# nanoporetech/bonito

Measured on AMD Instinct MI355X. Metric: signal samples/sec/GPU (chunk=10000, batch=512) + read accuracy vs ref, higher is better.
Workload: dtype f16

## Files before the change

### bonito_amd/csrc/conv.hip

```cpp
#include "common.h"
#include "kernels.h"
#include "options.h"
#include <cstring>

namespace bh {

struct ConvFirstArgs {
    const half_t* sig;
    const float* w;
    const float* bias;
    half_t* out;
    int N, Lin, Lout, Cout, K, stride, pad, act;
    float clamp_lo, clamp_hi;
    long os_n, os_t;
    int vec8;
};

__global__ __launch_bounds__(256) void conv_first_kernel(ConvFirstArgs p) {
    extern __shared__ __attribute__((aligned(16))) char smem[];
    float* wl = (float*)smem;
    float* bl = wl + p.Cout * p.K;
    float* sl = bl + p.Cout;
    const int n = blockIdx.y;
    const int tb = blockIdx.x * 256;
    const int span = 255 * p.stride + p.K;
    const half_t* s = p.sig + (long)n * p.Lin;
    for (int i = threadIdx.x; i < p.Cout * p.K; i += 256) wl[i] = p.w[i];
    for (int i = threadIdx.x; i < p.Cout; i += 256) bl[i] = p.bias ? p.bias[i] : 0.0f;
    for (int i = threadIdx.x; i < span; i += 256) {
        int pos = tb * p.stride - p.pad + i;
        sl[i] = (pos >= 0 && pos < p.Lin) ? (float)s[pos] : 0.0f;
    }
    __syncthreads();
    const int t = tb + threadIdx.x;
    if (t >= p.Lout) return;
    const float* x = sl + threadIdx.x * p.stride;
    half_t* dst = p.out + (long)n * p.os_n + (long)t * p.os_t;
    auto channel = [&](int c) {
        const float* wr = wl + c * p.K;
        float a = bl[c];
        for (int k = 0; k < p.K; ++k) a = fmaf(wr[k], x[k], a);
        a = apply_act_rt(a, p.act);
        return (half_t)fminf(fmaxf(a, p.clamp_lo), p.clamp_hi);
    };
    int c0 = 0;
    if (p.vec8) {
        if (p.K == 5 && p.act == ACT_SWISH) {
            const float x0 = x[0], x1 = x[1], x2 = x[2], x3 = x[3], x4 = x[4];
            for (; c0 + 8 <= p.Cout; c0 += 8) {
                half8_t o;
#pragma unroll
                for (int j = 0; j < 8; ++j) {
                    const float* wr = wl + (c0 + j) * 5;
                    float a = bl[c0 + j];
                    a = fmaf(wr[0], x0, a);
                    a = fmaf(wr[1], x1, a);
                    a = fmaf(wr[2], x2, a);
                    a = fmaf(wr[3], x3, a);
                    a = fmaf(wr[4], x4, a);
                    o[j] = (half_t)fminf(fmaxf(swishf_(a), p.clamp_lo), p.clamp_hi);
                }
                *(half8_t*)(dst + c0) = o;
            }
        }
        for (; c0 + 8 <= p.Cout; c0 += 8) {
            half8_t o;
#pragma unroll
            for (int j = 0; j < 8; ++j) o[j] = channel(c0 + j);
            *(half8_t*)(dst + c0) = o;
        }
    }
    for (; c0 < p.Cout; ++c0) dst[c0] = channel(c0);
}

struct ConvArgs {
    const half_t* in;
    const half_t* wpk;
    const float* bias;
    half_t* out;
    int N, Lin, Lout, Cin, Cout, K, stride, pad, act;
    int Kp;
    float clamp_lo, clamp_hi;
    long os_n, os_t;
};

template <int NTT, bool FS = false>
__global__ __launch_bounds__(256) void conv_igemm_kernel(ConvArgs p) {
    extern __shared__ __attribute__((aligned(16))) char smem[];
    half_t* xin = (half_t*)smem;
    constexpr int PW = NTT * 16;
    constexpr int PB = 4 * PW;
    const int tid = threadIdx.x, lane = tid & 63, wave = tid >> 6;
    const int r = lane & 15, kg = lane >> 4;
    const int n = blockIdx.y;
    const int t0 = blockIdx.x * PB;

    const int span_pos = (PB - 1) * p.stride + p.K;
    const int span_halves = span_pos * p.Cin + 32 + 8;
    const int p_start = t0 * p.stride - p.pad;
    const half_t* src = p.in + (long)n * p.Lin * p.Cin;
    for (int e = tid * 8; e < span_halves; e += 256 * 8) {
        int pos = p_start + e / p.Cin;
        uint4_t v = {0, 0, 0, 0};
        if (pos >= 0 && pos < p.Lin && e < span_pos * p.Cin)
            v = *(const uint4_t*)(src + (long)pos * p.Cin + (e % p.Cin));
        *(uint4_t*)(xin + e) = v;
    }
    __syncthreads();

    const int nks = p.Kp >> 5;
    const int nft = (p.Cout + 15) >> 4;
    constexpr int NT = FS ? 4 * NTT : NTT;
    const int pbase = FS ? 0 : wave * PW;
    int boff[NT];
#pragma unroll
    for (int tt = 0; tt < NT; ++tt)
        boff[tt] = (pbase + tt * 16 + r) * p.stride * p.Cin + kg * 8;

    for (int ft = FS ? wave : 0; ft < nft; ft += FS ? 4 : 1) {
        float4_t acc[NT];
#pragma unroll
        for (int tt = 0; tt < NT; ++tt) acc[tt] = float4_t{0.f, 0.f, 0.f, 0.f};
        const half_t* wrow = p.wpk + (long)(ft * 16 + r) * p.Kp + kg * 8;
        int ks = 0;
        for (; FS && ks + 4 <= nks; ks += 4) {
            half8_t a[4];
#pragma unroll
            for (int u = 0; u < 4; ++u) a[u] = *(const half8_t*)(wrow + (ks + u) * 32);
#pragma unroll
            for (int u = 0; u < 4; ++u)
#pragma unroll
                for (int tt = 0; tt < NT; ++tt) {
                    half8_t b = *(const half8_t*)(xin + boff[tt] + (ks + u) * 32);
                    acc[tt] = mfma16(a[u], b, acc[tt]);
                }
        }
        for (; ks < nks; ++ks) {
            half8_t a = *(const half8_t*)(wrow + ks * 32);
#pragma unroll
            for (int tt = 0; tt < NT; ++tt) {
                half8_t b = *(const half8_t*)(xin + boff[tt] + ks * 32);
                acc[tt] = mfma16(a, b, acc[tt]);
            }
        }
        const int f = ft * 16 + kg * 4;
        if (f < p.Cout) {
            float bv[4];
#pragma unroll
            for (int g = 0; g < 4; ++g) bv[g] = (p.bias && f + g < p.Cout) ? p.bias[f + g] : 0.0f;
#pragma unroll
            for (int tt = 0; tt < NT; ++tt) {
                int t = t0 + pbase + tt * 16 + r;
                if (t >= p.Lout) continue;
                float xv[4];
#pragma unroll
                for (int g = 0; g < 4; ++g) xv[g] = acc[tt][g] + bv[g];
                if (p.act == ACT_SWISH) {
#pragma unroll
                    for (int g = 0; g < 4; ++g) xv[g] = swishf_(xv[g]);
                } else {
#pragma unroll
                    for (int g = 0; g < 4; ++g) xv[g] = apply_act_rt(xv[g], p.act);
                }
                half4_t o;
#pragma unroll
                for (int g = 0; g < 4; ++g) o[g] = (half_t)fminf(fmaxf(xv[g], p.clamp_lo), p.clamp_hi);
                half_t* dst = p.out + (long)n * p.os_n + (long)t * p.os_t + f;
                if (f + 4 <= p.Cout) *(half4_t*)dst = o;
                else
                    for (int g = 0; g < 4; ++g)
                        if (f + g < p.Cout) dst[g] = o[g];
            }
        }
    }
}

template <int FPW, int NKS, int WAVES>
__global__ __launch_bounds__(64 * WAVES) void conv_ws_kernel(ConvArgs p) {
    extern __shared__ __attribute__((aligned(16))) char smem[];
    half_t* xin = (half_t*)smem;
    constexpr int PB = 256;
    const int tid = threadIdx.x, lane = tid & 63, wave = tid >> 6;
    const int r = lane & 15, kg = lane >> 4;
    const int n = blockIdx.y;
    const int t0 = blockIdx.x * PB;

    half8_t afr[FPW][NKS];
#pragma unroll
    for (int f = 0; f < FPW; ++f) {
        const half_t* wrow = p.wpk + (long)((wave * FPW + f) * 16 + r) * p.Kp + kg * 8;
#pragma unroll
        for (int ks = 0; ks < NKS; ++ks) afr[f][ks] = *(const half8_t*)(wrow + ks * 32);
    }
    float4_t bv[FPW];
#pragma unroll
    for (int f = 0; f < FPW; ++f) {
        bv[f] = float4_t{0.f, 0.f, 0.f, 0.f};
        if (p.bias) bv[f] = *(const float4_t*)(p.bias + (wave * FPW + f) * 16 + kg * 4);
    }

    const int span_pos = (PB - 1) * p.stride + p.K;
    const int span_halves = span_pos * p.Cin + 32 + 8;
    const int p_start = t0 * p.stride - p.pad;
    const half_t* src = p.in + (long)n * p.Lin * p.Cin;
    for (int e = tid * 8; e < span_halves; e += 64 * WAVES * 8) {
        int pos = p_start + e / p.Cin;
        uint4_t v = {0, 0, 0, 0};
        if (pos >= 0 && pos < p.Lin && e < span_pos * p.Cin)
            v = *(const uint4_t*)(src + (long)pos * p.Cin + (e % p.Cin));
        *(uint4_t*)(xin + e) = v;
    }
    __syncthreads();

    const int RS = p.stride * p.Cin;
    for (int pt = 0; pt < PB / 16; ++pt) {
        const int t = t0 + pt * 16 + r;
        if (t0 + pt * 16 >= p.Lout) break;
        const half_t* xrow = xin + (pt * 16 + r) * RS + kg * 8;
        half8_t b[NKS];
#pragma unroll
        for (int ks = 0; ks < NKS; ++ks) b[ks] = *(const half8_t*)(xrow + ks * 32);
        float4_t acc[FPW];
#pragma unroll
        for (int f = 0; f < FPW; ++f) acc[f] = float4_t{0.f, 0.f, 0.f, 0.f};
#pragma unroll
        for (int ks = 0; ks < NKS; ++ks)
#pragma unroll
            for (int f = 0; f < FPW; ++f) acc[f] = mfma16(afr[f][ks], b[ks], acc[f]);
#pragma unroll
        for (int f = 0; f < FPW; ++f)
#pragma unroll
            for (int g = 0; g < 4; ++g) acc[f][g] += bv[f][g];
        switch (p.act) {
            case ACT_SWISH:
#pragma unroll
                for (int f = 0; f < FPW; ++f)
#pragma unroll
                    for (int g = 0; g < 4; ++g) acc[f][g] = swishf_(acc[f][g]);
                break;
            case ACT_TANH:
#pragma unroll
                for (int f = 0; f < FPW; ++f)
#pragma unroll
                    for (int g = 0; g < 4; ++g) acc[f][g] = tanhf_(acc[f][g]);
                break;
            case ACT_RELU:
#pragma unroll
                for (int f = 0; f < FPW; ++f)
#pragma unroll
                    for (int g = 0; g < 4; ++g) acc[f][g] = fmaxf(acc[f][g], 0.0f);
                break;
            default: break;
        }
        if (t < p.Lout) {
            half_t* drow = p.out + (long)n * p.os_n + (long)t * p.os_t + kg * 4;
#pragma unroll
            for (int f = 0; f < FPW; ++f) {
                half4_t o;
#pragma unroll
                for (int g = 0; g < 4; ++g) o[g] = (half_t)fminf(fmaxf(acc[f][g], p.clamp_lo), p.clamp_hi);
                *(half4_t*)(drow + (wave * FPW + f) * 16) = o;
            }
        }
    }
}

struct ConvFront3Args {
    const half_t* sig;
    const float* w1;
    const float* b1;
    const half_t* w2pk;
    const float* b2;
    int L0, L1, L2;
    int K1, pad1, act1;
    int K2, pad2, act2;
    float lo1, hi1, lo2, hi2;
    ConvArgs c3;
};

template <int FPW, int NKS, int WAVES>
__global__ __launch_bounds__(64 * WAVES) void conv_front3_kernel(ConvFront3Args q) {
    extern __shared__ __attribute__((aligned(16))) char smem[];
    const ConvArgs& p = q.c3;
    constexpr int PB = 256, CH = 256, C16 = 16, NT = 64 * WAVES;
    const int tid = threadIdx.x, lane = tid & 63, wave = tid >> 6;
    const int r = lane & 15, kg = lane >> 4;
    const int n = blockIdx.y;
    const int t0 = blockIdx.x * PB;
    const int span_pos = (PB - 1) * p.stride + p.K;
    const int span_halves = span_pos * C16 + 32 + 8;
    half_t* xin = (half_t*)smem;
    half_t* a1 = xin + ((span_halves + 7) & ~7);
    const int a1_rows = CH + q.K2 - 1 + 6;
    float* sl = (float*)(a1 + a1_rows * C16);
    float* wl = sl + span_pos + q.K2 - 1 + q.K1 - 1 + 8;
    float* bl = wl + C16 * q.K1;

    half8_t a2[3];
#pragma unroll
    for (int ks = 0; ks < 3; ++ks) a2[ks] = *(const half8_t*)(q.w2pk + (long)r * 96 + kg * 8 + ks * 32);
    float b2v[4];
#pragma unroll
    for (int g = 0; g < 4; ++g) b2v[g] = q.b2 ? q.b2[kg * 4 + g] : 0.0f;

    const int p3_start = t0 * p.stride - p.pad;
    const int s_start = p3_start - q.pad2 - q.pad1;
    const int s_len = span_pos + q.K2 - 1 + q.K1 - 1;
    const half_t* sg = q.sig + (long)n * q.L0;
    for (int i = tid; i < s_len; i += NT) {
        const int pos = s_start + i;
        sl[i] = (pos >= 0 && pos < q.L0) ? (float)sg[pos] : 0.0f;
    }
    for (int i = tid; i < C16 * q.K1; i += NT) wl[i] = q.w1[i];
    if (tid < C16) bl[tid] = q.b1 ? q.b1[tid] : 0.0f;
    for (int e = span_pos * C16 + tid; e < span_halves; e += NT) xin[e] = (half_t)0.0f;
    for (int e = (CH + q.K2 - 1) * C16 + tid; e < a1_rows * C16; e += NT) a1[e] = (half_t)0.0f;
    __syncthreads();
    const int c0t = (tid & 1) * 8;
    float w1r[8][5], w1b[8];
    if (q.K1 == 5) {
#pragma unroll
        for (int c = 0; c < 8; ++c) {
            w1b[c] = bl[c0t + c];
#pragma unroll
            for (int k = 0; k < 5; ++k) w1r[c][k] = wl[(c0t + c) * 5 + k];
        }
    }

    for (int q0 = 0; q0 < span_pos; q0 += CH) {
        const int rows1 = min(CH, span_pos - q0) + q.K2 - 1;
        if (q.K1 == 5) {
            for (int w = tid; w < 2 * rows1; w += NT) {
                const int i = w >> 1;
                const int u = p3_start + q0 - q.pad2 + i;
                const float* x = sl + (q0 + i);
                const float x0 = x[0], x1 = x[1], x2 = x[2], x3 = x[3], x4 = x[4];
                float av[8];
#pragma unroll
                for (int c = 0; c < 8; ++c) {
                    float a = w1b[c];
                    a = fmaf(w1r[c][0], x0, a);
                    a = fmaf(w1r[c][1], x1, a);
                    a = fmaf(w1r[c][2], x2, a);
                    a = fmaf(w1r[c][3], x3, a);
                    a = fmaf(w1r[c][4], x4, a);
                    av[c] = a;
                }
                if (q.act1 == ACT_SWISH) {
#pragma unroll
                    for (int c = 0; c < 8; ++c) av[c] = swishf_(av[c]);
                } else {
#pragma unroll
                    for (int c = 0; c < 8; ++c) av[c] = apply_act_rt(av[c], q.act1);
                }
                const bool inside = u >= 0 && u < q.L1;
                half8_t o;
#pragma unroll
                for (int c = 0; c < 8; ++c) o[c] = inside ? (half_t)fminf(fmaxf(av[c], q.lo1), q.hi1) : (half_t)0.0f;
                *(half8_t*)(a1 + i * C16 + c0t) = o;
            }
        } else
        for (int w = tid; w < 2 * rows1; w += NT) {
            const int i = w >> 1, c0 = (w & 1) * 8;
            const int u = p3_start + q0 - q.pad2 + i;
            const float* x = sl + (q0 + i);
            half8_t o;
#pragma unroll
            for (int c = 0; c < 8; ++c) {
                const float* wr = wl + (c0 + c) * q.K1;
                float a = bl[c0 + c];
                for (int k = 0; k < q.K1; ++k) a = fmaf(wr[k], x[k], a);
                a = apply_act_rt(a, q.act1);
                const half_t hv = (half_t)fminf(fmaxf(a, q.lo1), q.hi1);
                o[c] = (u >= 0 && u < q.L1) ? hv : (half_t)0.0f;
            }
            *(half8_t*)(a1 + i * C16 + c0) = o;
        }
        __syncthreads();
        const int tiles = (min(CH, span_pos - q0) + 15) >> 4;
        for (int pt = wave; pt < tiles; pt += WAVES) {
            const half_t* xrow = a1 + (pt * 16 + r) * C16 + kg * 8;
            float4_t acc = {0.f, 0.f, 0.f, 0.f};
#pragma unroll
            for (int ks = 0; ks < 3; ++ks) acc = mfma16(a2[ks], *(const half8_t*)(xrow + ks * 32), acc);
            const int j = q0 + pt * 16 + r;
            const int v = p3_start + j;
            float xv[4];
#pragma unroll
            for (int g = 0; g < 4; ++g) xv[g] = acc[g] + b2v[g];
            if (q.act2 == ACT_SWISH) {
#pragma unroll
                for (int g = 0; g < 4; ++g) xv[g] = swishf_(xv[g]);
            } else {
#pragma unroll
                for (int g = 0; g < 4; ++g) xv[g] = apply_act_rt(xv[g], q.act2);
            }
            const bool inside = v >= 0 && v < q.L2;
            half4_t o;
#pragma unroll
            for (int g = 0; g < 4; ++g) o[g] = inside ? (half_t)fminf(fmaxf(xv[g], q.lo2), q.hi2) : (half_t)0.0f;
            if (j < span_pos) *(half4_t*)(xin + j * C16 + kg * 4) = o;
        }
        __syncthreads();
    }

    half8_t afr[FPW][NKS];
#pragma unroll
    for (int f = 0; f < FPW; ++f) {
        const half_t* wrow = p.wpk + (long)((wave * FPW + f) * 16 + r) * p.Kp + kg * 8;
#pragma unroll
        for (int ks = 0; ks < NKS; ++ks) afr[f][ks] = *(const half8_t*)(wrow + ks * 32);
    }
    float4_t bv[FPW];
#pragma unroll
    for (int f = 0; f < FPW; ++f) {
        bv[f] = float4_t{0.f, 0.f, 0.f, 0.f};
        if (p.bias) bv[f] = *(const float4_t*)(p.bias + (wave * FPW + f) * 16 + kg * 4);
    }
    const int RS = p.stride * C16;
    for (int pt = 0; pt < PB / 16; ++pt) {
        const int t = t0 + pt * 16 + r;
        if (t0 + pt * 16 >= p.Lout) break;
        const half_t* xrow = xin + (pt * 16 + r) * RS + kg * 8;
        half8_t b[NKS];
#pragma unroll
        for (int ks = 0; ks < NKS; ++ks) b[ks] = *(const half8_t*)(xrow + ks * 32);
        float4_t acc[FPW];
#pragma unroll
        for (int f = 0; f < FPW; ++f) acc[f] = float4_t{0.f, 0.f, 0.f, 0.f};
#pragma unroll
        for (int ks = 0; ks < NKS; ++ks)
#pragma unroll
            for (int f = 0; f < FPW; ++f) acc[f] = mfma16(afr[f][ks], b[ks], acc[f]);
#pragma unroll
        for (int f = 0; f < FPW; ++f)
#pragma unroll
            for (int g = 0; g < 4; ++g) acc[f][g] += bv[f][g];
        switch (p.act) {
            case ACT_SWISH:
#pragma unroll
                for (int f = 0; f < FPW; ++f)
#pragma unroll
                    for (int g = 0; g < 4; ++g) acc[f][g] = swishf_(acc[f][g]);
                break;
            case ACT_TANH:
#pragma unroll
                for (int f = 0; f < FPW; ++f)
#pragma unroll
                    for (int g = 0; g < 4; ++g) acc[f][g] = tanhf_(acc[f][g]);
                break;
            case ACT_RELU:
#pragma unroll
                for (int f = 0; f < FPW; ++f)
#pragma unroll
                    for (int g = 0; g < 4; ++g) acc[f][g] = fmaxf(acc[f][g], 0.0f);
                break;
            default: break;
        }
        if (t < p.Lout) {
            half_t* drow = p.out + (long)n * p.os_n + (long)t * p.os_t + kg * 4;
#pragma unroll
            for (int f = 0; f < FPW; ++f) {
                half4_t o;
#pragma unroll
                for (int g = 0; g < 4; ++g) o[g] = (half_t)fminf(fmaxf(acc[f][g], p.clamp_lo), p.clamp_hi);
#ifdef BH_CONV_EXPT_NOSTORE
                if (o[0] == (half_t)12345.0f)
#endif
                *(half4_t*)(drow + (wave * FPW + f) * 16) = o;
            }
        }
    }
}

}

int bh_k_conv_first(const void* signal, const float* w, const float* bias, void* out, int N, int Lin,
                    int Lout, int Cout, int K, int stride, int pad, int act, float clamp_lo,
                    float clamp_hi, long os_n, long os_t, hipStream_t stream) {
    using namespace bh;
    BH_REQUIRE(K >= 1 && Cout >= 1, "conv_first: bad shape (K=%d Cout=%d)", K, Cout);
    const int vec8 = (Cout % 8 == 0 && os_t % 8 == 0 && os_n % 8 == 0 && ((uintptr_t)out & 15) == 0) ? 1 : 0;
    ConvFirstArgs a{(const half_t*)signal, w, bias, (half_t*)out, N, Lin, Lout, Cout, K, stride, pad,
                    act, clamp_lo, clamp_hi, os_n, os_t, vec8};
    size_t lds = (size_t)(Cout * K + Cout + 255 * stride + K) * sizeof(float);
    hipLaunchKernelGGL(conv_first_kernel, dim3((Lout + 255) / 256, N), dim3(256), lds, stream, a);
    BH_CHECK_HIP(hipGetLastError());
    return 0;
}

int bh_k_conv_igemm(const void* in, const void* wpk, const float* bias, void* out, int N, int Lin,
                    int Lout, int Cin, int Cout, int K, int stride, int pad, int act, float clamp_lo,
                    float clamp_hi, long os_n, long os_t, hipStream_t stream) {
    using namespace bh;
    BH_REQUIRE(Cin % 8 == 0 && Cout % 4 == 0, "conv_igemm: need Cin%%8==0, Cout%%4==0 (Cin=%d Cout=%d)", Cin, Cout);
    BH_REQUIRE(os_t % 4 == 0 && os_n % 4 == 0, "conv_igemm: output strides must be multiples of 4");
    ConvArgs a{(const half_t*)in, (const half_t*)wpk, bias, (half_t*)out, N, Lin, Lout, Cin, Cout, K,
               stride, pad, act, ((K * Cin + 31) / 32) * 32, clamp_lo, clamp_hi, os_n, os_t};
    auto lds_for = [&](int pw) { return (size_t)(((4 * pw - 1) * stride + K) * Cin + 40) * 2 + 16; };
    if (bh::g_opt.conv_ws && (Cout == 384 || Cout == 96) && a.Kp == 320 && lds_for(64) <= 64 * 1024) {
        const dim3 wgrid((Lout + 255) / 256, N);
        if (Cout == 384) hipLaunchKernelGGL((conv_ws_kernel<3, 10, 8>), wgrid, dim3(512), lds_for(64), stream, a);
        else hipLaunchKernelGGL((conv_ws_kernel<1, 10, 6>), wgrid, dim3(384), lds_for(64), stream, a);
        BH_CHECK_HIP(hipGetLastError());
        return 0;
    }
    int pw = 64;
    while (pw > 16 && lds_for(pw) > (size_t)bh::g_opt.conv_lds_kb * 1024) pw >>= 1;
    size_t lds = lds_for(pw);
    BH_REQUIRE(lds <= 160 * 1024, "conv_igemm: input span does not fit LDS (%zu bytes)", lds);
    dim3 grid((Lout + 4 * pw - 1) / (4 * pw), N);
    if (lds > 64 * 1024) {
        const void* fn = pw == 64 ? (const void*)conv_igemm_kernel<4>
                         : pw == 32 ? (const void*)conv_igemm_kernel<2> : (const void*)conv_igemm_kernel<1>;
        BH_CHECK_HIP(bh_max_lds(fn, (int)lds));
    }
    const bool fs = bh::g_opt.conv_fs && Cout % 64 == 0;
    if (fs) {
        if (lds > 64 * 1024) {
            const void* fn = pw == 64 ? (const void*)conv_igemm_kernel<4, true>
                             : pw == 32 ? (const void*)conv_igemm_kernel<2, true> : (const void*)conv_igemm_kernel<1, true>;
            BH_CHECK_HIP(bh_max_lds(fn, (int)lds));
        }
        if (pw == 64) hipLaunchKernelGGL((conv_igemm_kernel<4, true>), grid, dim3(256), lds, stream, a);
        else if (pw == 32) hipLaunchKernelGGL((conv_igemm_kernel<2, true>), grid, dim3(256), lds, stream, a);
        else hipLaunchKernelGGL((conv_igemm_kernel<1, true>), grid, dim3(256), lds, stream, a);
    } else if (pw == 64) hipLaunchKernelGGL(conv_igemm_kernel<4>, grid, dim3(256), lds, stream, a);
    else if (pw == 32) hipLaunchKernelGGL(conv_igemm_kernel<2>, grid, dim3(256), lds, stream, a);
    else hipLaunchKernelGGL(conv_igemm_kernel<1>, grid, dim3(256), lds, stream, a);
    BH_CHECK_HIP(hipGetLastError());
    return 0;
}


int bh_k_conv_front3_ok(int c1_eff, int K1, int s1, int c2_in_eff, int c2_eff, int K2, int s2, int c3_in_eff, int c3_out, int K3, int s3) {
    if (!bh::g_opt.conv_fuse || !bh::g_opt.conv_ws) return 0;
    if (c1_eff != 16 || c2_in_eff != 16 || c2_eff != 16 || c3_in_eff != 16) return 0;
    if (s1 != 1 || s2 != 1 || K1 < 1 || K1 > 8 || K2 < 1 || K2 * 16 > 96) return 0;
    if (!(c3_out == 384 || c3_out == 96) || ((K3 * 16 + 31) / 32) * 32 != 320) return 0;
    if (c3_out == 96 && bh::g_opt.conv_fuse < 2) return 0;
    const size_t span = (size_t)255 * s3 + K3;
    const size_t lds = ((span * 16 + 40 + 7) & ~(size_t)7) * 2 + (size_t)(256 + K2 - 1 + 6) * 16 * 2 + (span + K2 + K1 + 6) * 4 + (size_t)(16 * K1 + 16) * 4;
    return lds <= 80 * 1024 ? 1 : 0;
}

int bh_k_conv_front3(const void* signal, int N, int L0, const float* w1, const float* b1, int K1, int pad1, int act1, float lo1, float hi1,
                     const void* w2pk, const float* b2, int K2, int pad2, int act2, float lo2, float hi2, const void* w3pk,
                     const float* b3, int Cout3, int K3, int stride3, int pad3, int act3, float lo3, float hi3, void* out, long os_n,
                     long os_t, hipStream_t stream) {
    using namespace bh;
    const int L1 = L0 + 2 * pad1 - K1 + 1, L2 = L1 + 2 * pad2 - K2 + 1, L3 = (L2 + 2 * pad3 - K3) / stride3 + 1;
    BH_REQUIRE(L1 > 0 && L2 > 0 && L3 > 0, "conv_front3: chunk of %d samples is too short", L0);
    BH_REQUIRE(os_t % 4 == 0 && os_n % 4 == 0, "conv_front3: output strides must be multiples of 4");
    ConvFront3Args a{(const half_t*)signal, w1, b1, (const half_t*)w2pk, b2, L0, L1, L2, K1, pad1, act1, K2, pad2, act2, lo1, hi1, lo2, hi2,
                     ConvArgs{nullptr, (const half_t*)w3pk, b3, (half_t*)out, N, L2, L3, 16, Cout3, K3, stride3, pad3, act3, 320, lo3, hi3,
                              os_n, os_t}};
    const size_t span = (size_t)255 * stride3 + K3;
    const size_t lds = ((span * 16 + 40 + 7) & ~(size_t)7) * 2 + (size_t)(256 + K2 - 1 + 6) * 16 * 2 + (span + K2 + K1 + 6) * 4 + (size_t)(16 * K1 + 16) * 4;
    const dim3 grid((L3 + 255) / 256, N);
    if (Cout3 == 384) {
        if (lds > 64 * 1024) BH_CHECK_HIP(bh_max_lds((const void*)conv_front3_kernel<3, 10, 8>, (int)lds));
        hipLaunchKernelGGL((conv_front3_kernel<3, 10, 8>), grid, dim3(512), lds, stream, a);
    } else {
        if (lds > 64 * 1024) BH_CHECK_HIP(bh_max_lds((const void*)conv_front3_kernel<1, 10, 6>, (int)lds));
        hipLaunchKernelGGL((conv_front3_kernel<1, 10, 6>), grid, dim3(384), lds, stream, a);
    }
    BH_CHECK_HIP(hipGetLastError());
    return 0;
}
```

### bonito_amd/csrc/options.cpp

```cpp
#include "options.h"

#include <string.h>

namespace bh {

Options g_opt;

#define BH_OPT(name) #name, &Options::name
static constexpr OptionRow OPTION_TABLE[] = {
    {BH_OPT(gemm_path), 0, Norm::keep, "linear GEMM kernel families: 0 auto, 1 = v1 only, 2 = no 256-tile kernel, 3 = no four-wave kernel, 5 = four-wave wherever legal"},
    {BH_OPT(gemm_tile16), 1, Norm::flag, "four-wave GEMM K-tile stream: 1 = 16x16x32 MFMAs, 0 = 32x32x16 (agree to fp16 rounding)"},
    {BH_OPT(gemm_order), 1, Norm::flag, "four-wave GEMM work order in an XCD: 1 = feature groups fastest, 0 = token blocks fastest (same bytes)"},
    {BH_OPT(gemm_gf), 0, Norm::keep, "four-wave GEMM feature tiles per block: 0 automatic, else rounded down to 1 / 2 / 4 / 8 / 16 / 32 (same bytes)"},
    {BH_OPT(gemm_stagger), 0, Norm::keep, "start-phase stagger of the persistent GEMM kernels, 0 = off (same bytes; measured without effect)"},
    {BH_OPT(attn_waves), 0, Norm::keep, "ring attention waves per workgroup: 0 automatic, 8, 12 (same results)"},
    {BH_OPT(attn_version), 2, Norm::one_or_two, "ring attention kernel: 2 = current, 1 = the first ring kernel"},
    {BH_OPT(attn_expt), 0, Norm::keep, "timing experiments of the ring attention kernel (bit mask): RESULTS ARE WRONG ON PURPOSE unless 0"},
    {BH_OPT(beam_fork), -1, Norm::keep, "posterior scan next to the beam kernel on a helper stream: -1 auto, 0 never, 1 always"},
    {BH_OPT(beam_select), 0, Norm::keep, "beam top-W selection: 0 histogram + boundary ranking, 1 radix search (same beams)"},
    {BH_OPT(beam_fuse), -1, Norm::keep, "forward / posterior scan as a second wave of the beam kernel: -1 auto (<= 256 states), 0 never, 1 always"},
    {BH_OPT(beam_cpw), 0, Norm::keep, "chunks per workgroup of the fused beam kernel at 256 states: 0 automatic, 1, 2, 4 (same bytes)"},
    {BH_OPT(decode_nt), 0, Norm::keep, "non-temporal score loads in the decode scans: 0 off"},
    {BH_OPT(viterbi_quad), 1, Norm::keep, "CRF Viterbi: 1 = four states per thread where the layout allows, 0 = the one-state kernel everywhere"},
    {BH_OPT(conv_ws), 1, Norm::keep, "weight-stationary kernel for the 384- / 96-channel 19-tap convolution: 1 on, 0 = generic implicit GEMM"},
    {BH_OPT(conv_fs), 1, Norm::keep, "feature-split instances of the implicit-GEMM convolution: 1 on, 0 = position-split"},
    {BH_OPT(conv_fuse), 1, Norm::keep, "conv1 -> conv2 -> conv3 as one kernel: 1 = 384-channel stacks, 2 = also 96-channel, 0 = three kernels"},
    {BH_OPT(conv_lds_kb), 64, Norm::positive_or_def, "KiB of LDS a workgroup of the implicit-GEMM convolution may take for its input span"},
    {BH_OPT(lstm_max_spins), 1000000, Norm::nonneg_or_def, "bound of the recurrent kernels' exchange spin loops (0: the first incomplete poll round is a timeout)"},
    {BH_OPT(lstm_q8_variant), 0, Norm::keep, "geometry of the 8-bit recurrent kernel, read at bh_encoder_create: 0, 1, 2"},
};
#undef BH_OPT

static constexpr bool defaults_agree() {
    constexpr Options o{};
    for (const OptionRow& r : OPTION_TABLE)
        if (o.*r.member != r.def) return false;
    return true;
}
static_assert(defaults_agree(), "options.h and OPTION_TABLE state different defaults");
static_assert(sizeof(OPTION_TABLE) / sizeof(OPTION_TABLE[0]) == sizeof(Options) / sizeof(int), "every member of Options has exactly one row");

const OptionRow* find_option(const char* name) {
    for (const OptionRow& r : OPTION_TABLE)
        if (!strcmp(name, r.name)) return &r;
    return nullptr;
}

}
```

### bonito_amd/csrc/options.h

```cpp
#pragma once

namespace bh {

struct Options {
    int gemm_path = 0;
    int gemm_tile16 = 1;
    int gemm_order = 1;
    int gemm_gf = 0;
    int gemm_stagger = 0;
    int attn_waves = 0;
    int attn_version = 2;
    int attn_expt = 0;
    int beam_fork = -1;
    int beam_select = 0;
    int beam_fuse = -1;
    int beam_cpw = 0;
    int decode_nt = 0;
    int viterbi_quad = 1;
    int conv_ws = 1;
    int conv_fs = 1;
    int conv_fuse = 1;
    int conv_lds_kb = 64;
    int lstm_max_spins = 1000000;
    int lstm_q8_variant = 0;
};
extern Options g_opt;

enum class Norm {
    keep,
    flag,
    one_or_two,
    positive_or_def,
    nonneg_or_def
};
struct OptionRow {
    const char* name;
    int Options::*member;
    int def;
    Norm norm;
    const char* what;
    int normalise(int v) const {
        switch (norm) {
            case Norm::flag: return v ? 1 : 0;
            case Norm::one_or_two: return v == 1 ? 1 : 2;
            case Norm::positive_or_def: return v > 0 ? v : def;
            case Norm::nonneg_or_def: return v >= 0 ? v : def;
            default: return v;
        }
    }
};
const OptionRow* find_option(const char* name);

}
```

Baseline: 342.2 million.

## Add three-pass fused conv front-end kernel computing whole span per workgroup

Adds a new conv1->conv2->conv3 fused kernel, specialised for K1=5 and swish, that runs three phases with barriers between them: first conv1 over the whole input span into LDS, then conv2 over that span with MFMAs, then conv3. The old kernel worked in 256-position chunks. The third stage software-pipelines its MFMA tiles against the epilogue and stores, and clamps use fmed3. It is on by default behind a new option, at the cost of more LDS per workgroup, which may lower occupancy.

```diff
diff --git a/bonito_amd/csrc/conv.hip b/bonito_amd/csrc/conv.hip
--- a/bonito_amd/csrc/conv.hip
+++ b/bonito_amd/csrc/conv.hip
@@ -473,6 +473,152 @@
     }
 }
 
+__device__ __forceinline__ float clampf_(float x, float lo, float hi) { return __builtin_amdgcn_fmed3f(x, lo, hi); }
+
+template <int FPW, int NKS, int WAVES, int ACT>
+__global__ __launch_bounds__(64 * WAVES) void conv_front3s_kernel(ConvFront3Args q) {
+    extern __shared__ __attribute__((aligned(16))) char smem[];
+    const ConvArgs& p = q.c3;
+    constexpr int PB = 256, C16 = 16, NT = 64 * WAVES;
+    const int tid = threadIdx.x, lane = tid & 63, wave = tid >> 6;
+    const int r = lane & 15, kg = lane >> 4;
+    const int n = blockIdx.y;
+    const int t0 = blockIdx.x * PB;
+    const int span_max = (PB - 1) * p.stride + p.K;
+    const int tiles3 = min(PB / 16, (p.Lout - t0 + 15) >> 4);
+    const int span_pos = (tiles3 * 16 - 1) * p.stride + p.K;
+    const int rows1 = span_pos + q.K2 - 1;
+    half_t* xin = (half_t*)smem;
+    half_t* a1 = xin + ((span_max * C16 + 32 + 8 + 7) & ~7);
+    float* sl = (float*)(a1 + (span_max + q.K2 - 1 + 6) * C16);
+    float* wl = sl + span_max + q.K2 - 1 + q.K1 - 1 + 8;
+    float* bl = wl + C16 * 5;
+
+    half8_t a2[3];
+#pragma unroll
+    for (int ks = 0; ks < 3; ++ks) a2[ks] = *(const half8_t*)(q.w2pk + (long)r * 96 + kg * 8 + ks * 32);
+    float b2v[4];
+#pragma unroll
+    for (int g = 0; g < 4; ++g) b2v[g] = q.b2 ? q.b2[kg * 4 + g] : 0.0f;
+
+    const int p3_start = t0 * p.stride - p.pad;
+    const int s_start = p3_start - q.pad2 - q.pad1;
+    const int s_len = rows1 + 5 - 1;
+    const half_t* sg = q.sig + (long)n * q.L0;
+    for (int i = tid; i < s_len; i += NT) {
+        const int pos = s_start + i;
+        sl[i] = (pos >= 0 && pos < q.L0) ? (float)sg[pos] : 0.0f;
+    }
+    for (int i = tid; i < C16 * 5; i += NT) wl[i] = q.w1[i];
+    if (tid < C16) bl[tid] = q.b1 ? q.b1[tid] : 0.0f;
+    for (int e = span_pos * C16 + tid; e < span_pos * C16 + 32 + 8; e += NT) xin[e] = (half_t)0.0f;
+    for (int e = rows1 * C16 + tid; e < (rows1 + 6) * C16; e += NT) a1[e] = (half_t)0.0f;
+    half8_t afr[FPW][NKS];
+#pragma unroll
+    for (int f = 0; f < FPW; ++f) {
+        const half_t* wrow = p.wpk + (long)((wave * FPW + f) * 16 + r) * p.Kp + kg * 8;
+#pragma unroll
+        for (int ks = 0; ks < NKS; ++ks) afr[f][ks] = *(const half8_t*)(wrow + ks * 32);
+    }
+    float4_t bv[FPW];
+#pragma unroll
+    for (int f = 0; f < FPW; ++f) {
+        bv[f] = float4_t{0.f, 0.f, 0.f, 0.f};
+        if (p.bias) bv[f] = *(const float4_t*)(p.bias + (wave * FPW + f) * 16 + kg * 4);
+    }
+    __syncthreads();
+
+    {
+        const int c0t = (tid & 1) * 8;
+        float w1r[8][5], w1b[8];
+#pragma unroll
+        for (int c = 0; c < 8; ++c) {
+            w1b[c] = bl[c0t + c];
+#pragma unroll
+            for (int k = 0; k < 5; ++k) w1r[c][k] = wl[(c0t + c) * 5 + k];
+        }
+        for (int w = tid; w < 2 * rows1; w += NT) {
+            const int i = w >> 1;
+            const int u = p3_start - q.pad2 + i;
+            const float* x = sl + i;
+            const float x0 = x[0], x1 = x[1], x2 = x[2], x3 = x[3], x4 = x[4];
+            const bool inside = u >= 0 && u < q.L1;
+            half8_t o;
+#pragma unroll
+            for (int c = 0; c < 8; ++c) {
+                float a = w1b[c];
+                a = fmaf(w1r[c][0], x0, a);
+                a = fmaf(w1r[c][1], x1, a);
+                a = fmaf(w1r[c][2], x2, a);
+                a = fmaf(w1r[c][3], x3, a);
+                a = fmaf(w1r[c][4], x4, a);
+                o[c] = inside ? (half_t)clampf_(apply_act<ACT>(a), q.lo1, q.hi1) : (half_t)0.0f;
+            }
+            *(half8_t*)(a1 + i * C16 + c0t) = o;
+        }
+    }
+    __syncthreads();
+
+    {
+        const int tiles2 = (span_pos + 15) >> 4;
+        for (int pt = wave; pt < tiles2; pt += WAVES) {
+            const half_t* xrow = a1 + (pt * 16 + r) * C16 + kg * 8;
+            float4_t acc = {0.f, 0.f, 0.f, 0.f};
+#pragma unroll
+            for (int ks = 0; ks < 3; ++ks) acc = mfma16(a2[ks], *(const half8_t*)(xrow + ks * 32), acc);
+            const int j = pt * 16 + r;
+            const int v = p3_start + j;
+            const bool inside = v >= 0 && v < q.L2;
+            half4_t o;
+#pragma unroll
+            for (int g = 0; g < 4; ++g) o[g] = inside ? (half_t)clampf_(apply_act<ACT>(acc[g] + b2v[g]), q.lo2, q.hi2) : (half_t)0.0f;
+            if (j < span_pos) *(half4_t*)(xin + j * C16 + kg * 4) = o;
+        }
+    }
+    __syncthreads();
+
+    const int RS = p.stride * C16;
+    auto mma = [&](int pt, float4_t (&acc)[FPW]) {
+        const half_t* xrow = xin + (pt * 16 + r) * RS + kg * 8;
+        half8_t b[NKS];
+#pragma unroll
+        for (int ks = 0; ks < NKS; ++ks) b[ks] = *(const half8_t*)(xrow + ks * 32);
+#pragma unroll
+        for (int f = 0; f < FPW; ++f) acc[f] = float4_t{0.f, 0.f, 0.f, 0.f};
+#pragma unroll
+        for (int ks = 0; ks < NKS; ++ks)
+#pragma unroll
+            for (int f = 0; f < FPW; ++f) acc[f] = mfma16(afr[f][ks], b[ks], acc[f]);
+    };
+    half_t* drow = p.out + (long)n * p.os_n + (long)(t0 + r) * p.os_t + kg * 4 + wave * FPW * 16;
+    const long dstep = 16 * p.os_t;
+    auto epilogue = [&](const float4_t (&acc)[FPW], half4_t (&o)[FPW]) {
+#pragma unroll
+        for (int f = 0; f < FPW; ++f)
+#pragma unroll
+            for (int g = 0; g < 4; ++g) o[f][g] = (half_t)clampf_(apply_act<ACT>(acc[f][g] + bv[f][g]), p.clamp_lo, p.clamp_hi);
+    };
+    const int full3 = min(tiles3, (p.Lout - t0) >> 4);
+    float4_t acc[FPW];
+    mma(0, acc);
+    for (int pt = 0; pt < full3; ++pt, drow += dstep) {
+        float4_t nxt[FPW];
+        mma(min(pt + 1, tiles3 - 1), nxt);
+        half4_t o[FPW];
+        epilogue(acc, o);
+#pragma unroll
+        for (int f = 0; f < FPW; ++f) *(half4_t*)(drow + f * 16) = o[f];
+#pragma unroll
+        for (int f = 0; f < FPW; ++f) acc[f] = nxt[f];
+    }
+    if (full3 < tiles3 && t0 + full3 * 16 + r < p.Lout) {
+        half4_t o[FPW];
+        epilogue(acc, o);
+#pragma unroll
+        for (int f = 0; f < FPW; ++f) *(half4_t*)(drow + f * 16) = o[f];
+    }
+}
+
 }
 
 int bh_k_conv_first(const void* signal, const float* w, const float* bias, void* out, int N, int Lin,
@@ -558,6 +704,19 @@
     const size_t span = (size_t)255 * stride3 + K3;
     const size_t lds = ((span * 16 + 40 + 7) & ~(size_t)7) * 2 + (size_t)(256 + K2 - 1 + 6) * 16 * 2 + (span + K2 + K1 + 6) * 4 + (size_t)(16 * K1 + 16) * 4;
     const dim3 grid((L3 + 255) / 256, N);
+    const size_t lds_s = ((span * 16 + 40 + 7) & ~(size_t)7) * 2 + (span + K2 - 1 + 6) * 16 * 2 + (span + K2 + K1 + 6) * 4 + (size_t)(16 * 5 + 16) * 4;
+    if (bh::g_opt.conv_front && K1 == 5 && act1 == ACT_SWISH && act2 == ACT_SWISH && act3 == ACT_SWISH && lo1 <= hi1 && lo2 <= hi2 &&
+        lo3 <= hi3 && lds_s <= 160 * 1024) {
+        if (Cout3 == 384) {
+            if (lds_s > 64 * 1024) BH_CHECK_HIP(bh_max_lds((const void*)conv_front3s_kernel<3, 10, 8, ACT_SWISH>, (int)lds_s));
+            hipLaunchKernelGGL((conv_front3s_kernel<3, 10, 8, ACT_SWISH>), grid, dim3(512), lds_s, stream, a);
+        } else {
+            if (lds_s > 64 * 1024) BH_CHECK_HIP(bh_max_lds((const void*)conv_front3s_kernel<1, 10, 6, ACT_SWISH>, (int)lds_s));
+            hipLaunchKernelGGL((conv_front3s_kernel<1, 10, 6, ACT_SWISH>), grid, dim3(384), lds_s, stream, a);
+        }
+        BH_CHECK_HIP(hipGetLastError());
+        return 0;
+    }
     if (Cout3 == 384) {
         if (lds > 64 * 1024) BH_CHECK_HIP(bh_max_lds((const void*)conv_front3_kernel<3, 10, 8>, (int)lds));
         hipLaunchKernelGGL((conv_front3_kernel<3, 10, 8>), grid, dim3(512), lds, stream, a);
diff --git a/bonito_amd/csrc/options.cpp b/bonito_amd/csrc/options.cpp
--- a/bonito_amd/csrc/options.cpp
+++ b/bonito_amd/csrc/options.cpp
@@ -25,6 +25,7 @@
     {BH_OPT(conv_ws), 1, Norm::keep, "weight-stationary kernel for the 384- / 96-channel 19-tap convolution: 1 on, 0 = generic implicit GEMM"},
     {BH_OPT(conv_fs), 1, Norm::keep, "feature-split instances of the implicit-GEMM convolution: 1 on, 0 = position-split"},
     {BH_OPT(conv_fuse), 1, Norm::keep, "conv1 -> conv2 -> conv3 as one kernel: 1 = 384-channel stacks, 2 = also 96-channel, 0 = three kernels"},
+    {BH_OPT(conv_front), 1, Norm::flag, "fused conv front end: 1 = whole span in three passes, 0 = chunks of 256 positions (same bytes)"},
     {BH_OPT(conv_lds_kb), 64, Norm::positive_or_def, "KiB of LDS a workgroup of the implicit-GEMM convolution may take for its input span"},
     {BH_OPT(lstm_max_spins), 1000000, Norm::nonneg_or_def, "bound of the recurrent kernels' exchange spin loops (0: the first incomplete poll round is a timeout)"},
     {BH_OPT(lstm_q8_variant), 0, Norm::keep, "geometry of the 8-bit recurrent kernel, read at bh_encoder_create: 0, 1, 2"},
diff --git a/bonito_amd/csrc/options.h b/bonito_amd/csrc/options.h
--- a/bonito_amd/csrc/options.h
+++ b/bonito_amd/csrc/options.h
@@ -20,6 +20,7 @@
     int conv_ws = 1;
     int conv_fs = 1;
     int conv_fuse = 1;
+    int conv_front = 1;
     int conv_lds_kb = 64;
     int lstm_max_spins = 1000000;
     int lstm_q8_variant = 0;
```

Result: no change. 342.8 million (median of 6 runs) (+0.2%).
